# yilunliao/vit-search

Hardware: AMD Instinct MI355X
Metric: images/sec/node ViT-ResNAS-Tiny supernet train, bs128/GPU, 1/2/4/8 MI355X (higher is better)
Workload: dtype bf16

## Files before the change

vit-search_amd/csrc/attn_mfma.hip:

```cpp
#include <cstdlib>

#include "common.h"
#include "../../include/vitres_hip.h"

namespace vr_attn_mfma {

typedef __bf16 bfv8 __attribute__((ext_vector_type(8)));

template <int D> struct AC {
    static constexpr int NCH = D / 8;
    static constexpr int DK = (D + 31) / 32;
    static constexpr int DT = D / 16;
    static constexpr bool SWZ = (D != 48);
};

template <typename TI = bf16_t> __device__ __forceinline__ f32x4 mfma16(bfv8 a, bfv8 b, f32x4 c) { return Half16<TI>::mfma16(a, b, c); }

template <int D, int MAXNP, int NTHR>
__device__ __forceinline__ void stage_chunked(char* dst, const bf16_t* __restrict__ src, int rs, int N, int Np, int tid) {
    const int NpS = Np + 8;
    constexpr int NCH = AC<D>::NCH, HP = NCH / 2;
    constexpr int IT = (MAXNP * NCH + NTHR - 1) / NTHR;
    const int total = Np * NCH;
    uint4 v[IT];
// ... 71 lines not shown
    __device__ static __forceinline__ int tbase(int lane) {
        const int g = lane >> 4, i = lane & 15;
        return ((((i & 3) >> 1)) * (NP + 8) + 4 * g + (i >> 2)) * 16 + (i & 1) * 8;
    }
    __device__ static __forceinline__ const char* opaque(const char* p) {
        typedef __attribute__((address_space(3))) const char lds_char;
        unsigned a = (unsigned)(unsigned long long)(lds_char*)p;
        asm volatile("" : "+v"(a));
        return (const char*)(lds_char*)(unsigned long long)a;
    }
    __device__ static __forceinline__ bfv8 cread(const char* lane_base, int row0) {
        return *reinterpret_cast<const bfv8*>(lane_base + row0 * 16);
    }
    __device__ static __forceinline__ bfv8 tread(const char* lane_base, int kp, int dt) {
        typedef __attribute__((address_space(3))) s4v lds_s4v;
        const char* p = lane_base + (2 * dt * (NP + 8) + 32 * kp) * 16;
        const s4v lo = __builtin_amdgcn_ds_read_tr16_b64_v4i16((lds_s4v*)(p));
        const s4v hi = __builtin_amdgcn_ds_read_tr16_b64_v4i16((lds_s4v*)(p + 16 * 16));
        const s8v v = {lo[0], lo[1], lo[2], lo[3], hi[0], hi[1], hi[2], hi[3]};
        return __builtin_bit_cast(bfv8, v);
    }
};

template <int D, int NKP, int NW, int PB, int OCC, bool FULL, typename TI = bf16_t>
__global__ __launch_bounds__(NW * 64, OCC) void fwd_kernel(const bf16_t* __restrict__ qkv, bf16_t* __restrict__ o,
                                                           float* __restrict__ lse, const int* __restrict__ keep_hd, int B,
                                                           int N, int H, float scale, int ATTN_XCD) {
    static_assert(NKP % PB == 0, "key-tile pairs must split into whole blocks");
    constexpr int NP = 32 * NKP;
    typedef Img<D, NP> I;
    extern __shared__ __attribute__((aligned(16))) char sm[];
    const int bidx = xcd_block((int)blockIdx.x, (int)gridDim.x, ATTN_XCD);
    const int b = bidx / H, h = bidx % H;
    const int tid = threadIdx.x, lane = tid & 63, wave = tid >> 6, g = lane >> 4, c = lane & 15;
    const int HD = H * D, RS = 3 * HD;
    const bf16_t* base = qkv + (long long)b * N * RS + h * D;
    bf16_t* ob = o + (long long)b * N * HD + h * D;
    float* lb = lse + ((long long)b * H + h) * N;
    if (keep_hd && h * D >= keep_hd[b]) {
        for (int i = tid; i < N * (D / 8); i += NW * 64) {
            const int n = i / (D / 8), ch = i % (D / 8);
            *reinterpret_cast<uint4*>(ob + (long long)n * HD + ch * 8) = make_uint4(0, 0, 0, 0);
        }
        for (int n = tid; n < N; n += NW * 64) lb[n] = 0.f;
        return;
    }
    char* Kc = sm;
    char* Vc = sm + I::BYTES;
    int q0 = wave * 16;
    bfv8 qf[AC<D>::DK];
#pragma unroll
    for (int dk = 0; dk < AC<D>::DK; ++dk) qf[dk] = gfrag<D>(base, RS, q0, N, dk, lane);
    stage_chunked<D, NP, NW * 64>(Kc, base + HD, RS, N, NP, tid);
    stage_chunked<D, NP, NW * 64>(Vc, base + 2 * HD, RS, N, NP, tid);
    __syncthreads();
    const char* kb[AC<D>::DK];
#pragma unroll
    for (int dk = 0; dk < AC<D>::DK; ++dk) kb[dk] = I::opaque(Kc + I::cbase(dk, lane));
    const char* vb = I::opaque(Vc + I::tbase(lane));
    const float cs = scale * LOG2E;
    while (q0 < N) {
        float m = -INFINITY, sum = 0.f;
        f32x4 oacc[AC<D>::DT];
#pragma unroll
        for (int dt = 0; dt < AC<D>::DT; ++dt) oacc[dt] = f32x4{0.f, 0.f, 0.f, 0.f};
#pragma unroll
        for (int b0 = 0; b0 < NKP; b0 += PB) {
            if (FULL || b0 * 32 < N) {
                f32x4 st[2 * PB];
                float bm = -INFINITY;
#pragma unroll
                for (int j = 0; j < 2 * PB; ++j) {
                    const int k0 = (2 * b0 + j) * 16;
                    f32x4 acc = {0.f, 0.f, 0.f, 0.f};
                    if (FULL || k0 < N) {
#pragma unroll
                        for (int dk = 0; dk < AC<D>::DK; ++dk) acc = mfma16<TI>(I::cread(kb[dk], k0), qf[dk], acc);
                        if (FULL ? (2 * b0 + j >= 2 * NKP - 2) : (k0 + 16 > N)) {
#pragma unroll
                            for (int r = 0; r < 4; ++r) acc[r] = (k0 + 4 * g + r) < N ? acc[r] : -INFINITY;
                        }
                    } else {
                        acc = f32x4{-INFINITY, -INFINITY, -INFINITY, -INFINITY};
                    }
                    st[j] = acc;
                    bm = fmaxf(fmaxf(bm, fmaxf(acc[0], acc[1])), fmaxf(acc[2], acc[3]));
                }
                bm = gmax(bm);
                const float mn = fmaxf(m, bm);
                const float alpha = ex2((m - mn) * cs);
                const float mc = mn * cs;
                float ps = 0.f;
#pragma unroll
                for (int j = 0; j < 2 * PB; ++j)
#pragma unroll
                    for (int r = 0; r < 4; ++r) {
                        const float pv = ex2(fmaf(st[j][r], cs, -mc));
                        st[j][r] = pv;
                        ps += pv;
                    }
                sum = sum * alpha + ps;
                m = mn;
                if (b0 > 0) {
#pragma unroll
                    for (int dt = 0; dt < AC<D>::DT; ++dt)
#pragma unroll
                        for (int r = 0; r < 4; ++r) oacc[dt][r] *= alpha;
                }
#pragma unroll
                for (int jp = 0; jp < PB; ++jp) {
                    if (FULL || (b0 + jp) * 32 < N) {
                        const bfv8 pf = pack8<TI>(st[2 * jp], st[2 * jp + 1]);
#pragma unroll
                        for (int dt = 0; dt < AC<D>::DT; ++dt) oacc[dt] = mfma16<TI>(I::tread(vb, b0 + jp, dt), pf, oacc[dt]);
                    }
                }
                __builtin_amdgcn_sched_barrier(0);
            }
        }
        sum = gsum(sum);
        const float inv = 1.0f / sum;
        const int qs = q0;
        q0 += NW * 16;
        bfv8 qn[AC<D>::DK];
        if (q0 < N) {
#pragma unroll
            for (int dk = 0; dk < AC<D>::DK; ++dk) qn[dk] = gfrag<D>(base, RS, q0, N, dk, lane);
        }
        if (qs + c < N) {
#pragma unroll
            for (int dt = 0; dt < AC<D>::DT; ++dt)
                *reinterpret_cast<uint2*>(ob + (long long)(qs + c) * HD + dt * 16 + 4 * g) =
                    make_uint2(Half16<TI>::pk(oacc[dt][0] * inv, oacc[dt][1] * inv), Half16<TI>::pk(oacc[dt][2] * inv, oacc[dt][3] * inv));
            if (g == 0) lb[qs + c] = m * scale + __logf(sum);
        }
        if (q0 < N) {
#pragma unroll
            for (int dk = 0; dk < AC<D>::DK; ++dk) qf[dk] = qn[dk];
        }
    }
}

template <int D, int NKP, int NW, int OCC, bool FULL>
__global__ __launch_bounds__(NW * 64, OCC) void bwd_dq_kernel(const bf16_t* __restrict__ qkv, const bf16_t* __restrict__ o,
                                                              const bf16_t* __restrict__ d_o, const float* __restrict__ lse,
                                                              float* __restrict__ delta, bf16_t* __restrict__ dqkv,
                                                              const int* __restrict__ keep_hd, int B, int N, int H,
                                                              float scale, int ATTN_XCD) {
    constexpr int NP = 32 * NKP;
    typedef Img<D, NP> I;
    extern __shared__ __attribute__((aligned(16))) char sm[];
    const int bidx = xcd_block((int)blockIdx.x, (int)gridDim.x, ATTN_XCD);
    const int b = bidx / H, h = bidx % H;
    const int tid = threadIdx.x, lane = tid & 63, wave = tid >> 6, g = lane >> 4, c = lane & 15;
    const int HD = H * D, RS = 3 * HD;
    const bf16_t* base = qkv + (long long)b * N * RS + h * D;
    bf16_t* dbase = dqkv + (long long)b * N * RS + h * D;
    if (keep_hd && h * D >= keep_hd[b]) {
        for (int i = tid; i < N * (D / 8); i += NW * 64) {
            const int n = i / (D / 8), ch = i % (D / 8);
            *reinterpret_cast<uint4*>(dbase + (long long)n * RS + ch * 8) = make_uint4(0, 0, 0, 0);
        }
        return;
    }
    const bf16_t* ob = o + (long long)b * N * HD + h * D;
    const bf16_t* gb = d_o + (long long)b * N * HD + h * D;
    const float* lb = lse + ((long long)b * H + h) * N;
    float* db = delta + ((long long)b * H + h) * N;
    char* Kc = sm;
    char* Vc = Kc + I::BYTES;
    int q0 = wave * 16;
    bfv8 qf[AC<D>::DK], gf[AC<D>::DK], of[AC<D>::DK];
    float lq = 0.f;
#pragma unroll
    for (int dk = 0; dk < AC<D>::DK; ++dk) {
        qf[dk] = gfrag<D>(base, RS, q0, N, dk, lane);
        gf[dk] = gfrag<D>(gb, HD, q0, N, dk, lane);
        of[dk] = gfrag<D>(ob, HD, q0, N, dk, lane);
    }
    if (q0 + c < N) lq = lb[q0 + c];
    stage_chunked<D, NP, NW * 64>(Kc, base + HD, RS, N, NP, tid);
    stage_chunked<D, NP, NW * 64>(Vc, base + 2 * HD, RS, N, NP, tid);
    __syncthreads();
    const char *kb[AC<D>::DK], *vb[AC<D>::DK];
#pragma unroll
    for (int dk = 0; dk < AC<D>::DK; ++dk) {
        kb[dk] = I::opaque(Kc + I::cbase(dk, lane));
        vb[dk] = I::opaque(Vc + I::cbase(dk, lane));
    }
    const char* kt_b = I::opaque(Kc + I::tbase(lane));
    const float cs = scale * LOG2E;
    while (q0 < N) {
        float d = 0.f;
#pragma unroll
        for (int dk = 0; dk < AC<D>::DK; ++dk)
#pragma unroll
            for (int e = 0; e < 8; ++e) d += (float)gf[dk][e] * (float)of[dk][e];
        const float dl = gsum(d);
        const float l2 = lq * LOG2E;
        if (g == 0 && q0 + c < N) db[q0 + c] = dl;
        f32x4 dq[AC<D>::DT];
#pragma unroll
        for (int dt = 0; dt < AC<D>::DT; ++dt) dq[dt] = f32x4{0.f, 0.f, 0.f, 0.f};
#pragma unroll
        for (int kp = 0; kp < NKP; ++kp) {
            if (FULL || kp * 32 < N) {
                f32x4 ds[2];
#pragma unroll
                for (int tt = 0; tt < 2; ++tt) {
                    const int k0 = (2 * kp + tt) * 16;
                    f32x4 sc = {0.f, 0.f, 0.f, 0.f}, dp = {0.f, 0.f, 0.f, 0.f};
                    if (FULL || k0 < N) {
#pragma unroll
                        for (int dk = 0; dk < AC<D>::DK; ++dk) {
                            sc = mfma16(I::cread(kb[dk], k0), qf[dk], sc);
                            dp = mfma16(I::cread(vb[dk], k0), gf[dk], dp);
                        }
#pragma unroll
                        for (int r = 0; r < 4; ++r) sc[r] = ex2(fmaf(sc[r], cs, -l2)) * ((dp[r] - dl) * scale);
                    }
                    ds[tt] = sc;
                }
                const bfv8 sf = pack8(ds[0], ds[1]);
#pragma unroll
                for (int dt = 0; dt < AC<D>::DT; ++dt) dq[dt] = mfma16(I::tread(kt_b, kp, dt), sf, dq[dt]);
                if (kp % 3 == 2) __builtin_amdgcn_sched_barrier(0);
            }
        }
        const int qs = q0;
        q0 += NW * 16;
        if (q0 < N) {
#pragma unroll
            for (int dk = 0; dk < AC<D>::DK; ++dk) {
                qf[dk] = gfrag<D>(base, RS, q0, N, dk, lane);
                gf[dk] = gfrag<D>(gb, HD, q0, N, dk, lane);
                of[dk] = gfrag<D>(ob, HD, q0, N, dk, lane);
            }
            lq = q0 + c < N ? lb[q0 + c] : 0.f;
        }
        if (qs + c < N) {
#pragma unroll
            for (int dt = 0; dt < AC<D>::DT; ++dt)
                *reinterpret_cast<uint2*>(dbase + (long long)(qs + c) * RS + dt * 16 + 4 * g) =
                    make_uint2(pack_bf2(dq[dt][0], dq[dt][1]), pack_bf2(dq[dt][2], dq[dt][3]));
        }
    }
}

template <int D, int NKP, int NW, int OCC, bool FULL>
__global__ __launch_bounds__(NW * 64, OCC) void bwd_dkv_kernel(const bf16_t* __restrict__ qkv, const bf16_t* __restrict__ d_o,
                                                               const float* __restrict__ lse, const float* __restrict__ delta,
                                                               bf16_t* __restrict__ dqkv, const int* __restrict__ keep_hd,
                                                               int B, int N, int H, float scale, int ATTN_XCD) {
    constexpr int NP = 32 * NKP;
    typedef Img<D, NP> I;
    extern __shared__ __attribute__((aligned(16))) char sm[];
    const int bidx = xcd_block((int)blockIdx.x, (int)gridDim.x, ATTN_XCD);
    const int b = bidx / H, h = bidx % H;
    const int tid = threadIdx.x, lane = tid & 63, wave = tid >> 6, g = lane >> 4, c = lane & 15;
    const int HD = H * D, RS = 3 * HD;
    const bf16_t* base = qkv + (long long)b * N * RS + h * D;
    bf16_t* dbase = dqkv + (long long)b * N * RS + h * D;
    if (keep_hd && h * D >= keep_hd[b]) {
        for (int i = tid; i < N * (D / 8); i += NW * 64) {
            const int n = i / (D / 8), ch = i % (D / 8);
            *reinterpret_cast<uint4*>(dbase + (long long)n * RS + HD + ch * 8) = make_uint4(0, 0, 0, 0);
            *reinterpret_cast<uint4*>(dbase + (long long)n * RS + 2 * HD + ch * 8) = make_uint4(0, 0, 0, 0);
        }
        return;
    }
    const bf16_t* gb = d_o + (long long)b * N * HD + h * D;
    const int nqp = FULL ? NKP : (N + 31) / 32;
    char* Qc = sm;
    char* Gc = Qc + I::BYTES;
    float* Ls = reinterpret_cast<float*>(Gc + I::BYTES);
    float* Ds = Ls + NP;
    int u0 = wave * 16;
    bfv8 kf[AC<D>::DK], vf[AC<D>::DK];
#pragma unroll
    for (int dk = 0; dk < AC<D>::DK; ++dk) {
        kf[dk] = gfrag<D>(base + HD, RS, u0, N, dk, lane);
        vf[dk] = gfrag<D>(base + 2 * HD, RS, u0, N, dk, lane);
    }
    for (int n = tid; n < NP; n += NW * 64) {
        Ls[n] = n < N ? lse[((long long)b * H + h) * N + n] * LOG2E : 0.f;
        Ds[n] = n < N ? delta[((long long)b * H + h) * N + n] : 0.f;
    }
    stage_chunked<D, NP, NW * 64>(Qc, base, RS, N, NP, tid);
    stage_chunked<D, NP, NW * 64>(Gc, gb, HD, N, NP, tid);
    __syncthreads();
    const char *qb[AC<D>::DK], *gcb[AC<D>::DK];
#pragma unroll
    for (int dk = 0; dk < AC<D>::DK; ++dk) {
        qb[dk] = I::opaque(Qc + I::cbase(dk, lane));
        gcb[dk] = I::opaque(Gc + I::cbase(dk, lane));
    }
    const char* qt_b = I::opaque(Qc + I::tbase(lane));
    const char* gt_b = I::opaque(Gc + I::tbase(lane));
    const float* lsg = Ls + 4 * g;
    const float* dsg = Ds + 4 * g;
    const float cs = scale * LOG2E;
    while (u0 < N) {
        f32x4 dka[AC<D>::DT], dva[AC<D>::DT];
#pragma unroll
        for (int dt = 0; dt < AC<D>::DT; ++dt) {
            dka[dt] = f32x4{0.f, 0.f, 0.f, 0.f};
            dva[dt] = f32x4{0.f, 0.f, 0.f, 0.f};
        }
#pragma unroll(NKP <= 3 ? NKP : 1)
        for (int qp = 0; qp < nqp; ++qp) {
            f32x4 p[2], ds[2];
#pragma unroll
            for (int tt = 0; tt < 2; ++tt) {
                const int q0 = qp * 32 + tt * 16;
                const float4 l4 = *reinterpret_cast<const float4*>(lsg + q0);
                const float4 d4 = *reinterpret_cast<const float4*>(dsg + q0);
                const float lr[4] = {l4.x, l4.y, l4.z, l4.w}, dr[4] = {d4.x, d4.y, d4.z, d4.w};
                f32x4 sc = {0.f, 0.f, 0.f, 0.f}, dp = {0.f, 0.f, 0.f, 0.f};
#pragma unroll
                for (int dk = 0; dk < AC<D>::DK; ++dk) {
                    sc = mfma16(I::cread(qb[dk], q0), kf[dk], sc);
                    dp = mfma16(I::cread(gcb[dk], q0), vf[dk], dp);
                }
#pragma unroll
                for (int r = 0; r < 4; ++r) {
                    const float pv = ex2(fmaf(sc[r], cs, -lr[r]));
                    p[tt][r] = pv;
                    ds[tt][r] = pv * ((dp[r] - dr[r]) * scale);
                }
            }
            const bfv8 pf = pack8(p[0], p[1]), sf = pack8(ds[0], ds[1]);
#pragma unroll
            for (int dt = 0; dt < AC<D>::DT; ++dt) {
                dva[dt] = mfma16(I::tread(gt_b, qp, dt), pf, dva[dt]);
                dka[dt] = mfma16(I::tread(qt_b, qp, dt), sf, dka[dt]);
            }
            __builtin_amdgcn_sched_barrier(0);
        }
        const int k = u0 + c;
        u0 += NW * 16;
        if (u0 < N) {
#pragma unroll
            for (int dk = 0; dk < AC<D>::DK; ++dk) {
                kf[dk] = gfrag<D>(base + HD, RS, u0, N, dk, lane);
                vf[dk] = gfrag<D>(base + 2 * HD, RS, u0, N, dk, lane);
            }
        }
        if (k < N) {
#pragma unroll
            for (int dt = 0; dt < AC<D>::DT; ++dt) {
                bf16_t* dst = dbase + (long long)k * RS + dt * 16 + 4 * g;
                *reinterpret_cast<uint2*>(dst + HD) =
                    make_uint2(pack_bf2(dka[dt][0], dka[dt][1]), pack_bf2(dka[dt][2], dka[dt][3]));
                *reinterpret_cast<uint2*>(dst + 2 * HD) =
                    make_uint2(pack_bf2(dva[dt][0], dva[dt][1]), pack_bf2(dva[dt][2], dva[dt][3]));
            }
        }
    }
}

template <int D, int MAXNP, int NTHR>
__device__ __forceinline__ void stage_load(uint4 (&v)[(MAXNP * AC<D>::NCH + NTHR - 1) / NTHR], const bf16_t* __restrict__ src, int rs,
                                           int N, int Np, int tid) {
    constexpr int NCH = AC<D>::NCH, HP = NCH / 2;
    constexpr int IT = (MAXNP * NCH + NTHR - 1) / NTHR;
    const int total = Np * NCH;
#pragma unroll
    for (int it = 0; it < IT; ++it) {
        const int idx = tid + it * NTHR;
        const int q = idx >> 3, l8 = idx & 7;
        const int rb = q / HP, cp = q - rb * HP;
        const int n = 4 * rb + (l8 >> 1), ch = 2 * cp + (l8 & 1);
        const bool ok = n < N && idx < total;
        v[it] = *reinterpret_cast<const uint4*>(src + (long long)(ok ? n : 0) * rs + (ok ? ch : 0) * 8);
        if (!ok) v[it] = make_uint4(0, 0, 0, 0);
    }
}
template <int D, int MAXNP, int NTHR>
__device__ __forceinline__ void stage_store(char* dst, const uint4 (&v)[(MAXNP * AC<D>::NCH + NTHR - 1) / NTHR], int Np, int tid) {
    const int NpS = Np + 8;
    constexpr int NCH = AC<D>::NCH, HP = NCH / 2;
    constexpr int IT = (MAXNP * NCH + NTHR - 1) / NTHR;
    const int total = Np * NCH;
#pragma unroll
    for (int it = 0; it < IT; ++it) {
        const int idx = tid + it * NTHR;
        const int q = idx >> 3, l8 = idx & 7;
        const int rb = q / HP, cp = q - rb * HP;
        const int n = 4 * rb + (l8 >> 1), ch = 2 * cp + (l8 & 1);
        if (idx < total) *reinterpret_cast<uint4*>(dst + ((size_t)ch * NpS + n) * 16) = v[it];
    }
}

template <int D, int NKP, int NW, int OCC, bool FULL>
__global__ __launch_bounds__(NW * 64, OCC) void bwd_short_kernel(const bf16_t* __restrict__ qkv, const bf16_t* __restrict__ o,
                                                                 const bf16_t* __restrict__ d_o, const float* __restrict__ lse,
                                                                 float* __restrict__ delta, bf16_t* __restrict__ dqkv,
                                                                 const int* __restrict__ keep_hd, int B, int N, int H,
                                                                 float scale, int ATTN_XCD) {
    constexpr int NP = 32 * NKP, NT = NW * 64;
    constexpr int IT = (NP * AC<D>::NCH + NT - 1) / NT;
    typedef Img<D, NP> I;
    extern __shared__ __attribute__((aligned(16))) char sm[];
    const int bidx = xcd_block((int)blockIdx.x, (int)gridDim.x, ATTN_XCD);
    const int b = bidx / H, h = bidx % H;
    const int tid = threadIdx.x, lane = tid & 63, wave = tid >> 6, g = lane >> 4, c = lane & 15;
    const int HD = H * D, RS = 3 * HD;
    const bf16_t* base = qkv + (long long)b * N * RS + h * D;
    bf16_t* dbase = dqkv + (long long)b * N * RS + h * D;
    if (keep_hd && h * D >= keep_hd[b]) {
        for (int i = tid; i < N * (D / 8); i += NT) {
            const int n = i / (D / 8), ch = i % (D / 8);
            bf16_t* dst = dbase + (long long)n * RS + ch * 8;
            *reinterpret_cast<uint4*>(dst) = make_uint4(0, 0, 0, 0);
            *reinterpret_cast<uint4*>(dst + HD) = make_uint4(0, 0, 0, 0);
            *reinterpret_cast<uint4*>(dst + 2 * HD) = make_uint4(0, 0, 0, 0);
        }
        return;
    }
    const bf16_t* ob = o + (long long)b * N * HD + h * D;
    const bf16_t* gb = d_o + (long long)b * N * HD + h * D;
    const float* lb = lse + ((long long)b * H + h) * N;
// ... 24 lines not shown
        stage_store<D, NP, NT>(Gc, vg, NP, tid);
    }
    __syncthreads();
    const char *qb[AC<D>::DK], *kb[AC<D>::DK], *vb[AC<D>::DK], *gcb[AC<D>::DK];
#pragma unroll
    for (int dk = 0; dk < AC<D>::DK; ++dk) {
        qb[dk] = I::opaque(Qc + I::cbase(dk, lane));
        kb[dk] = I::opaque(Kc + I::cbase(dk, lane));
        vb[dk] = I::opaque(Vc + I::cbase(dk, lane));
        gcb[dk] = I::opaque(Gc + I::cbase(dk, lane));
    }
    const char* kt_b = I::opaque(Kc + I::tbase(lane));
    const char* qt_b = I::opaque(Qc + I::tbase(lane));
    const char* gt_b = I::opaque(Gc + I::tbase(lane));
    const float cs = scale * LOG2E;
    auto zfrag = [&](const char* lane_base, int row0, int dk) -> bfv8 {
        bfv8 v = I::cread(lane_base, row0);
        if constexpr (AC<D>::NCH % 4 != 0) {
            if (dk * 4 + (lane >> 4) >= AC<D>::NCH) v = __builtin_bit_cast(bfv8, make_uint4(0, 0, 0, 0));
        }
        return v;
    };

    while (q0 < N) {
        bfv8 qf[AC<D>::DK], gf[AC<D>::DK];
#pragma unroll
        for (int dk = 0; dk < AC<D>::DK; ++dk) {
            qf[dk] = zfrag(qb[dk], q0, dk);
            gf[dk] = zfrag(gcb[dk], q0, dk);
        }
        float d = 0.f;
#pragma unroll
        for (int dk = 0; dk < AC<D>::DK; ++dk)
#pragma unroll
            for (int e = 0; e < 8; ++e) d += (float)gf[dk][e] * (float)of[dk][e];
        const float dl = gsum(d);
        const float l2 = Ls[q0 + c];
        if (g == 0 && q0 + c < N) {
            db[q0 + c] = dl;
            Ds[q0 + c] = dl;
        }
        f32x4 dq[AC<D>::DT];
#pragma unroll
        for (int dt = 0; dt < AC<D>::DT; ++dt) dq[dt] = f32x4{0.f, 0.f, 0.f, 0.f};
#pragma unroll
        for (int kp = 0; kp < NKP; ++kp) {
            if (FULL || kp * 32 < N) {
                f32x4 ds[2];
#pragma unroll
                for (int tt = 0; tt < 2; ++tt) {
                    const int k0 = (2 * kp + tt) * 16;
                    f32x4 sc = {0.f, 0.f, 0.f, 0.f}, dp = {0.f, 0.f, 0.f, 0.f};
                    if (FULL || k0 < N) {
#pragma unroll
                        for (int dk = 0; dk < AC<D>::DK; ++dk) {
                            sc = mfma16(I::cread(kb[dk], k0), qf[dk], sc);
                            dp = mfma16(I::cread(vb[dk], k0), gf[dk], dp);
                        }
#pragma unroll
                        for (int r = 0; r < 4; ++r) sc[r] = ex2(fmaf(sc[r], cs, -l2)) * ((dp[r] - dl) * scale);
                    }
                    ds[tt] = sc;
                }
                const bfv8 sf = pack8(ds[0], ds[1]);
#pragma unroll
                for (int dt = 0; dt < AC<D>::DT; ++dt) dq[dt] = mfma16(I::tread(kt_b, kp, dt), sf, dq[dt]);
                __builtin_amdgcn_sched_barrier(0);
            }
        }
        const int qs = q0;
        q0 += NW * 16;
        if (q0 < N) {
#pragma unroll
            for (int dk = 0; dk < AC<D>::DK; ++dk) of[dk] = gfrag<D>(ob, HD, q0, N, dk, lane);
        }
        if (qs + c < N) {
#pragma unroll
            for (int dt = 0; dt < AC<D>::DT; ++dt)
                *reinterpret_cast<uint2*>(dbase + (long long)(qs + c) * RS + dt * 16 + 4 * g) =
                    make_uint2(pack_bf2(dq[dt][0], dq[dt][1]), pack_bf2(dq[dt][2], dq[dt][3]));
        }
    }
    __syncthreads();

    const int nqp = FULL ? NKP : (N + 31) / 32;
    const float* lsg = Ls + 4 * g;
    const float* dsg = Ds + 4 * g;
    for (int u0 = wave * 16; u0 < N; u0 += NW * 16) {
        bfv8 kf[AC<D>::DK], vf[AC<D>::DK];
#pragma unroll
        for (int dk = 0; dk < AC<D>::DK; ++dk) {
            kf[dk] = zfrag(kb[dk], u0, dk);
            vf[dk] = zfrag(vb[dk], u0, dk);
        }
        f32x4 dka[AC<D>::DT], dva[AC<D>::DT];
#pragma unroll
        for (int dt = 0; dt < AC<D>::DT; ++dt) {
            dka[dt] = f32x4{0.f, 0.f, 0.f, 0.f};
            dva[dt] = f32x4{0.f, 0.f, 0.f, 0.f};
        }
#pragma unroll
        for (int qp = 0; qp < NKP; ++qp) {
            if (qp < nqp) {
                f32x4 p[2], ds[2];
#pragma unroll
                for (int tt = 0; tt < 2; ++tt) {
                    const int qq = qp * 32 + tt * 16;
                    const float4 l4 = *reinterpret_cast<const float4*>(lsg + qq);
                    const float4 d4 = *reinterpret_cast<const float4*>(dsg + qq);
                    const float lr[4] = {l4.x, l4.y, l4.z, l4.w}, dr[4] = {d4.x, d4.y, d4.z, d4.w};
                    f32x4 sc = {0.f, 0.f, 0.f, 0.f}, dp = {0.f, 0.f, 0.f, 0.f};
#pragma unroll
                    for (int dk = 0; dk < AC<D>::DK; ++dk) {
                        sc = mfma16(I::cread(qb[dk], qq), kf[dk], sc);
                        dp = mfma16(I::cread(gcb[dk], qq), vf[dk], dp);
                    }
#pragma unroll
                    for (int r = 0; r < 4; ++r) {
                        const float pv = ex2(fmaf(sc[r], cs, -lr[r]));
                        p[tt][r] = pv;
                        ds[tt][r] = pv * ((dp[r] - dr[r]) * scale);
                    }
                }
                const bfv8 pf = pack8(p[0], p[1]), sf = pack8(ds[0], ds[1]);
#pragma unroll
                for (int dt = 0; dt < AC<D>::DT; ++dt) {
                    dva[dt] = mfma16(I::tread(gt_b, qp, dt), pf, dva[dt]);
                    dka[dt] = mfma16(I::tread(qt_b, qp, dt), sf, dka[dt]);
                }
                __builtin_amdgcn_sched_barrier(0);
            }
        }
        const int k = u0 + c;
        if (k < N) {
#pragma unroll
            for (int dt = 0; dt < AC<D>::DT; ++dt) {
                bf16_t* dst = dbase + (long long)k * RS + dt * 16 + 4 * g;
                *reinterpret_cast<uint2*>(dst + HD) =
                    make_uint2(pack_bf2(dka[dt][0], dka[dt][1]), pack_bf2(dka[dt][2], dka[dt][3]));
                *reinterpret_cast<uint2*>(dst + 2 * HD) =
                    make_uint2(pack_bf2(dva[dt][0], dva[dt][1]), pack_bf2(dva[dt][2], dva[dt][3]));
            }
        }
    }
}

constexpr int LKB = 256, LQB = 128, LNW = 8;

template <int D, typename TI = bf16_t>
__global__ __launch_bounds__(LNW * 64) void fwd_long_kernel(const bf16_t* __restrict__ qkv, bf16_t* __restrict__ o,
                                                            float* __restrict__ lse, const int* __restrict__ keep_hd, int B,
                                                            int N, int H, float scale) {
    extern __shared__ __attribute__((aligned(16))) char sm[];
    const int nqb = (N + LQB - 1) / LQB;
    const int qb = blockIdx.x % nqb, bh = blockIdx.x / nqb, b = bh / H, h = bh % H;
    const int tid = threadIdx.x, lane = tid & 63, wave = tid >> 6, g = lane >> 4, c = lane & 15;
    const int HD = H * D, RS = 3 * HD;
    const bf16_t* base = qkv + (long long)b * N * RS + h * D;
    bf16_t* ob = o + (long long)b * N * HD + h * D;
    float* lb = lse + ((long long)b * H + h) * N;
    const int q0 = qb * LQB + wave * 16;
    if (keep_hd && h * D >= keep_hd[b]) {
        for (int i = tid; i < LQB * (D / 8); i += LNW * 64) {
            const int n = qb * LQB + i / (D / 8), ch = i % (D / 8);
            if (n < N) *reinterpret_cast<uint4*>(ob + (long long)n * HD + ch * 8) = make_uint4(0, 0, 0, 0);
        }
// ... 249 lines not shown
            *reinterpret_cast<uint2*>(dst + 2 * HD) = make_uint2(pack_bf2(dva[dt][0], dva[dt][1]), pack_bf2(dva[dt][2], dva[dt][3]));
        }
    }
}

template <typename K> static int set_lds(K kernel, size_t bytes) {
    static size_t granted = 0;
    if (bytes > 64 * 1024 && bytes > granted) {
        hipError_t e = hipFuncSetAttribute(reinterpret_cast<const void*>(kernel), hipFuncAttributeMaxDynamicSharedMemorySize,
                                           (int)bytes);
        if (e != hipSuccess) return (int)e;
        granted = bytes;
    }
    return 0;
}

template <int NKP> struct Plan {
    static constexpr int NW = NKP >= 9 ? 8 : 4;
    static constexpr int OCC = 4;
    static constexpr int PB = NKP >= 9 ? 3 : NKP;
};

static constexpr int attn_xcd() { return 1; }
template <int D, int NKP, typename TI = bf16_t>
static int launch_fwd(const bf16_t* qkv, bf16_t* o, float* lse, const int* keep, int B, int N, int H, float scale,
                      hipStream_t st) {
    constexpr int NW = Plan<NKP>::NW, OCC = Plan<NKP>::OCC, PB = Plan<NKP>::PB;
    const size_t lds = (size_t)2 * Img<D, 32 * NKP>::BYTES;
    if (N > 32 * (NKP - 1)) {
        int rc = set_lds(fwd_kernel<D, NKP, NW, PB, OCC, true, TI>, lds);
        if (rc) return rc;
        hipLaunchKernelGGL((fwd_kernel<D, NKP, NW, PB, OCC, true, TI>), dim3(B * H), dim3(NW * 64), lds, st, qkv, o, lse, keep, B, N, H,
                           scale, attn_xcd());
    } else {
        int rc = set_lds(fwd_kernel<D, NKP, NW, PB, OCC, false, TI>, lds);
        if (rc) return rc;
        hipLaunchKernelGGL((fwd_kernel<D, NKP, NW, PB, OCC, false, TI>), dim3(B * H), dim3(NW * 64), lds, st, qkv, o, lse, keep, B, N, H,
                           scale, attn_xcd());
    }
    return 0;
}
template <int D, int NKP>
static int launch_bwd(const bf16_t* qkv, const bf16_t* o, const bf16_t* d_o, const float* lse, float* delta, bf16_t* dqkv,
                      const int* keep, int B, int N, int H, float scale, hipStream_t st) {
    constexpr int NW = Plan<NKP>::NW, OCC = Plan<NKP>::OCC;
    const size_t l1 = (size_t)2 * Img<D, 32 * NKP>::BYTES, l2 = l1 + 2 * 32 * NKP * sizeof(float);
    {
        constexpr size_t L3 = (size_t)4 * Img<D, 32 * NKP>::BYTES + 2 * 32 * NKP * sizeof(float);
        constexpr int SOCC = NKP <= 3 ? 3 : (L3 <= 80 * 1024 ? 2 : 1);
        const bool merged = SOCC >= 2;
        if (merged) {
            const size_t l3 = (size_t)4 * Img<D, 32 * NKP>::BYTES + 2 * 32 * NKP * sizeof(float);
            if (N > 32 * (NKP - 1)) {
                int rc = set_lds(bwd_short_kernel<D, NKP, NW, SOCC, true>, l3);
                if (rc) return rc;
                hipLaunchKernelGGL((bwd_short_kernel<D, NKP, NW, SOCC, true>), dim3(B * H), dim3(NW * 64), l3, st, qkv, o, d_o, lse, delta,
                                   dqkv, keep, B, N, H, scale, attn_xcd());
            } else {
                int rc = set_lds(bwd_short_kernel<D, NKP, NW, SOCC, false>, l3);
                if (rc) return rc;
                hipLaunchKernelGGL((bwd_short_kernel<D, NKP, NW, SOCC, false>), dim3(B * H), dim3(NW * 64), l3, st, qkv, o, d_o, lse, delta,
                                   dqkv, keep, B, N, H, scale, attn_xcd());
            }
            return 0;
        }
    }
    if (N > 32 * (NKP - 1)) {
        int rc = set_lds(bwd_dq_kernel<D, NKP, NW, OCC, true>, l1);
        if (rc) return rc;
        rc = set_lds(bwd_dkv_kernel<D, NKP, NW, OCC, true>, l2);
        if (rc) return rc;
        hipLaunchKernelGGL((bwd_dq_kernel<D, NKP, NW, OCC, true>), dim3(B * H), dim3(NW * 64), l1, st, qkv, o, d_o, lse, delta, dqkv,
                           keep, B, N, H, scale, attn_xcd());
        hipLaunchKernelGGL((bwd_dkv_kernel<D, NKP, NW, OCC, true>), dim3(B * H), dim3(NW * 64), l2, st, qkv, d_o, lse, delta, dqkv,
                           keep, B, N, H, scale, attn_xcd());
    } else {
        int rc = set_lds(bwd_dq_kernel<D, NKP, NW, OCC, false>, l1);
        if (rc) return rc;
        rc = set_lds(bwd_dkv_kernel<D, NKP, NW, OCC, false>, l2);
        if (rc) return rc;
        hipLaunchKernelGGL((bwd_dq_kernel<D, NKP, NW, OCC, false>), dim3(B * H), dim3(NW * 64), l1, st, qkv, o, d_o, lse, delta, dqkv,
                           keep, B, N, H, scale, attn_xcd());
        hipLaunchKernelGGL((bwd_dkv_kernel<D, NKP, NW, OCC, false>), dim3(B * H), dim3(NW * 64), l2, st, qkv, d_o, lse, delta, dqkv,
                           keep, B, N, H, scale, attn_xcd());
    }
    return 0;
}

template <int D, typename TI = bf16_t>
static int launch_fwd_long(const bf16_t* qkv, bf16_t* o, float* lse, const int* keep, int B, int N, int H, float scale,
                           hipStream_t st) {
    const size_t lds = (size_t)2 * D * (LKB + 8) * 2;
    int rc = set_lds(fwd_long_kernel<D, TI>, lds);
    if (rc) return rc;
    hipLaunchKernelGGL((fwd_long_kernel<D, TI>), dim3(B * H * ((N + LQB - 1) / LQB)), dim3(LNW * 64), lds, st, qkv, o, lse, keep, B, N, H,
                       scale);
    return 0;
}
template <int D>
static int launch_bwd_long(const bf16_t* qkv, const bf16_t* o, const bf16_t* d_o, const float* lse, float* delta, bf16_t* dqkv,
                           const int* keep, int B, int N, int H, float scale, hipStream_t st) {
    const size_t l1 = (size_t)2 * D * (LKB + 8) * 2, l2 = l1 + 2 * LKB * sizeof(float);
    int rc = set_lds(bwd_dq_long_kernel<D>, l1);
    if (rc) return rc;
    rc = set_lds(bwd_dkv_long_kernel<D>, l2);
    if (rc) return rc;
    const unsigned grid = (unsigned)(B * H * ((N + LQB - 1) / LQB));
    hipLaunchKernelGGL((bwd_dq_long_kernel<D>), dim3(grid), dim3(LNW * 64), l1, st, qkv, o, d_o, lse, delta, dqkv, keep, B, N, H, scale);
// ... 62 lines not shown
```

Baseline: 18660.

## Specialize attention kernels for partial last key tile and single-row tail

Adds MODE template specializations for the attention forward and backward kernels based on how many rows fall in the last 32-wide tile. When that tile holds at most 16 rows, the upper 16-row half is skipped entirely. When only one row is left (e.g. a CLS token making N = 32k+1), that row is handled by a dedicated tail path split across waves and reduced through LDS, so the main loop stops at a 16-aligned boundary. This removes wasted MFMA and exp work on padded tiles, at the cost of extra syncthreads, LDS reductions and more template instances.

New measurement: 18640. No clear change (-0.1%).

```diff
diff --git a/vit-search_amd/csrc/attn_mfma.hip b/vit-search_amd/csrc/attn_mfma.hip
--- a/vit-search_amd/csrc/attn_mfma.hip
+++ b/vit-search_amd/csrc/attn_mfma.hip
@@ -1,4 +1,5 @@
 #include <cstdlib>
+#include <type_traits>
 
 #include "common.h"
 #include "../../include/vitres_hip.h"
@@ -117,11 +118,102 @@
     }
 };
 
-template <int D, int NKP, int NW, int PB, int OCC, bool FULL, typename TI = bf16_t>
+template <int MODE> struct Mode {
+    static constexpr bool FULL = MODE >= 1, HALF = MODE >= 2, TAIL = MODE == 3;
+};
+template <int D, int NROW>
+__device__ __forceinline__ void tail_put(float* P, int wave, int slot, const f32x4 (&acc)[AC<D>::DT], int g, int c) {
+    if (c == 0) {
+#pragma unroll
+        for (int dt = 0; dt < AC<D>::DT; ++dt)
+            *reinterpret_cast<float4*>(P + (wave * NROW + slot) * D + dt * 16 + 4 * g) = make_float4(acc[dt][0], acc[dt][1], acc[dt][2], acc[dt][3]);
+    }
+}
+template <int D, int NROW, int NW>
+__device__ __forceinline__ void tail_sum_store(const float* P, bf16_t* dst, int sst, int tid) {
+    if (tid < NROW * D / 2) {
+        const int slot = tid / (D / 2), d = 2 * (tid % (D / 2));
+        float a0 = 0.f, a1 = 0.f;
+#pragma unroll
+        for (int w = 0; w < NW; ++w) {
+            const float2 v = *reinterpret_cast<const float2*>(P + (w * NROW + slot) * D + d);
+            a0 += v.x;
+            a1 += v.y;
+        }
+        *reinterpret_cast<uint32_t*>(dst + slot * sst + d) = pack_bf2(a0, a1);
+    }
+}
+template <int D, int NKP, int NW, typename I>
+__device__ __forceinline__ void tail_dq(f32x4 (&dq)[AC<D>::DT], const bfv8 (&qf)[AC<D>::DK], const bfv8 (&gf)[AC<D>::DK], float l2, float dl,
+                                        const char* const (&kb)[AC<D>::DK], const char* const (&vb)[AC<D>::DK], const char* kt_b,
+                                        float cs, float scale, int wave) {
+    for (int kp = wave; kp < NKP; kp += NW) {
+        f32x4 ds[2];
+#pragma unroll
+        for (int tt = 0; tt < 2; ++tt) {
+            f32x4 sc = {0.f, 0.f, 0.f, 0.f}, dp = {0.f, 0.f, 0.f, 0.f};
+            if (tt == 0 || kp != NKP - 1) {
+                const int k0 = (2 * kp + tt) * 16;
+#pragma unroll
+                for (int dk = 0; dk < AC<D>::DK; ++dk) {
+                    sc = mfma16(I::cread(kb[dk], k0), qf[dk], sc);
+                    dp = mfma16(I::cread(vb[dk], k0), gf[dk], dp);
+                }
+#pragma unroll
+                for (int r = 0; r < 4; ++r) sc[r] = ex2(fmaf(sc[r], cs, -l2)) * ((dp[r] - dl) * scale);
+            }
+            ds[tt] = sc;
+        }
+        const bfv8 sf = pack8(ds[0], ds[1]);
+#pragma unroll
+        for (int dt = 0; dt < AC<D>::DT; ++dt) dq[dt] = mfma16(I::tread(kt_b, kp, dt), sf, dq[dt]);
+    }
+}
+template <int D, int NKP, int NW, typename I>
+__device__ __forceinline__ void tail_dkv(f32x4 (&dka)[AC<D>::DT], f32x4 (&dva)[AC<D>::DT], const bfv8 (&kf)[AC<D>::DK],
+                                         const bfv8 (&vf)[AC<D>::DK], const char* const (&qb)[AC<D>::DK],
+                                         const char* const (&gcb)[AC<D>::DK], const char* qt_b, const char* gt_b, const float* lsg,
+                                         const float* dsg, float cs, float scale, int wave) {
+    for (int qp = wave; qp < NKP; qp += NW) {
+        f32x4 p[2], ds[2];
+#pragma unroll
+        for (int tt = 0; tt < 2; ++tt) {
+            p[tt] = f32x4{0.f, 0.f, 0.f, 0.f};
+            ds[tt] = f32x4{0.f, 0.f, 0.f, 0.f};
+            if (tt == 0 || qp != NKP - 1) {
+                const int q0 = qp * 32 + tt * 16;
+                const float4 l4 = *reinterpret_cast<const float4*>(lsg + q0);
+                const float4 d4 = *reinterpret_cast<const float4*>(dsg + q0);
+                const float lr[4] = {l4.x, l4.y, l4.z, l4.w}, dr[4] = {d4.x, d4.y, d4.z, d4.w};
+                f32x4 sc = {0.f, 0.f, 0.f, 0.f}, dp = {0.f, 0.f, 0.f, 0.f};
+#pragma unroll
+                for (int dk = 0; dk < AC<D>::DK; ++dk) {
+                    sc = mfma16(I::cread(qb[dk], q0), kf[dk], sc);
+                    dp = mfma16(I::cread(gcb[dk], q0), vf[dk], dp);
+                }
+#pragma unroll
+                for (int r = 0; r < 4; ++r) {
+                    const float pv = ex2(fmaf(sc[r], cs, -lr[r]));
+                    p[tt][r] = pv;
+                    ds[tt][r] = pv * ((dp[r] - dr[r]) * scale);
+                }
+            }
+        }
+        const bfv8 pf = pack8(p[0], p[1]), sf = pack8(ds[0], ds[1]);
+#pragma unroll
+        for (int dt = 0; dt < AC<D>::DT; ++dt) {
+            dva[dt] = mfma16(I::tread(gt_b, qp, dt), pf, dva[dt]);
+            dka[dt] = mfma16(I::tread(qt_b, qp, dt), sf, dka[dt]);
+        }
+    }
+}
+
+template <int D, int NKP, int NW, int PB, int OCC, int MODE, typename TI = bf16_t>
 __global__ __launch_bounds__(NW * 64, OCC) void fwd_kernel(const bf16_t* __restrict__ qkv, bf16_t* __restrict__ o,
                                                            float* __restrict__ lse, const int* __restrict__ keep_hd, int B,
                                                            int N, int H, float scale, int ATTN_XCD) {
     static_assert(NKP % PB == 0, "key-tile pairs must split into whole blocks");
+    constexpr bool FULL = Mode<MODE>::FULL, HALF = Mode<MODE>::HALF, TAIL = Mode<MODE>::TAIL;
     constexpr int NP = 32 * NKP;
     typedef Img<D, NP> I;
     extern __shared__ __attribute__((aligned(16))) char sm[];
@@ -154,7 +246,8 @@
     for (int dk = 0; dk < AC<D>::DK; ++dk) kb[dk] = I::opaque(Kc + I::cbase(dk, lane));
     const char* vb = I::opaque(Vc + I::tbase(lane));
     const float cs = scale * LOG2E;
-    while (q0 < N) {
+    const int NE = TAIL ? N - 1 : N;
+    while (q0 < NE) {
         float m = -INFINITY, sum = 0.f;
         f32x4 oacc[AC<D>::DT];
 #pragma unroll
@@ -168,10 +261,14 @@
                 for (int j = 0; j < 2 * PB; ++j) {
                     const int k0 = (2 * b0 + j) * 16;
                     f32x4 acc = {0.f, 0.f, 0.f, 0.f};
+                    if (HALF && 2 * b0 + j == 2 * NKP - 1) {
+                        st[j] = acc;
+                        continue;
+                    }
                     if (FULL || k0 < N) {
 #pragma unroll
                         for (int dk = 0; dk < AC<D>::DK; ++dk) acc = mfma16<TI>(I::cread(kb[dk], k0), qf[dk], acc);
-                        if (FULL ? (2 * b0 + j >= 2 * NKP - 2) : (k0 + 16 > N)) {
+                        if (HALF ? (2 * b0 + j == 2 * NKP - 2) : FULL ? (2 * b0 + j >= 2 * NKP - 2) : (k0 + 16 > N)) {
 #pragma unroll
                             for (int r = 0; r < 4; ++r) acc[r] = (k0 + 4 * g + r) < N ? acc[r] : -INFINITY;
                         }
@@ -187,13 +284,15 @@
                 const float mc = mn * cs;
                 float ps = 0.f;
 #pragma unroll
-                for (int j = 0; j < 2 * PB; ++j)
+                for (int j = 0; j < 2 * PB; ++j) {
+                    if (HALF && 2 * b0 + j == 2 * NKP - 1) continue;
 #pragma unroll
                     for (int r = 0; r < 4; ++r) {
                         const float pv = ex2(fmaf(st[j][r], cs, -mc));
                         st[j][r] = pv;
                         ps += pv;
                     }
+                }
                 sum = sum * alpha + ps;
                 m = mn;
                 if (b0 > 0) {
@@ -218,7 +317,7 @@
         const int qs = q0;
         q0 += NW * 16;
         bfv8 qn[AC<D>::DK];
-        if (q0 < N) {
+        if (q0 < NE) {
 #pragma unroll
             for (int dk = 0; dk < AC<D>::DK; ++dk) qn[dk] = gfrag<D>(base, RS, q0, N, dk, lane);
         }
@@ -229,19 +328,96 @@
                     make_uint2(Half16<TI>::pk(oacc[dt][0] * inv, oacc[dt][1] * inv), Half16<TI>::pk(oacc[dt][2] * inv, oacc[dt][3] * inv));
             if (g == 0) lb[qs + c] = m * scale + __logf(sum);
         }
-        if (q0 < N) {
+        if (q0 < NE) {
 #pragma unroll
             for (int dk = 0; dk < AC<D>::DK; ++dk) qf[dk] = qn[dk];
         }
     }
-}
-
-template <int D, int NKP, int NW, int OCC, bool FULL>
+    if constexpr (TAIL) {
+#pragma unroll
+        for (int dk = 0; dk < AC<D>::DK; ++dk) qf[dk] = gfrag<D>(base, RS, N - 1, N, dk, lane);
+        float m = -INFINITY, sum = 0.f;
+        f32x4 oacc[AC<D>::DT];
+#pragma unroll
+        for (int dt = 0; dt < AC<D>::DT; ++dt) oacc[dt] = f32x4{0.f, 0.f, 0.f, 0.f};
+        for (int kp = wave; kp < NKP; kp += NW) {
+            f32x4 s0 = {0.f, 0.f, 0.f, 0.f}, s1 = {0.f, 0.f, 0.f, 0.f};
+            const bool last = kp == NKP - 1;
+#pragma unroll
+            for (int dk = 0; dk < AC<D>::DK; ++dk) s0 = mfma16<TI>(I::cread(kb[dk], 32 * kp), qf[dk], s0);
+            float bm;
+            if (last) {
+#pragma unroll
+                for (int r = 0; r < 4; ++r) s0[r] = (32 * kp + 4 * g + r) < N ? s0[r] : -INFINITY;
+                bm = fmaxf(fmaxf(s0[0], s0[1]), fmaxf(s0[2], s0[3]));
+            } else {
+#pragma unroll
+                for (int dk = 0; dk < AC<D>::DK; ++dk) s1 = mfma16<TI>(I::cread(kb[dk], 32 * kp + 16), qf[dk], s1);
+                bm = fmaxf(fmaxf(fmaxf(s0[0], s0[1]), fmaxf(s0[2], s0[3])), fmaxf(fmaxf(s1[0], s1[1]), fmaxf(s1[2], s1[3])));
+            }
+            bm = gmax(bm);
+            const float mn = fmaxf(m, bm);
+            const float alpha = ex2((m - mn) * cs);
+            const float mc = mn * cs;
+            float ps = 0.f;
+#pragma unroll
+            for (int r = 0; r < 4; ++r) {
+                s0[r] = ex2(fmaf(s0[r], cs, -mc));
+                ps += s0[r];
+            }
+            if (!last) {
+#pragma unroll
+                for (int r = 0; r < 4; ++r) {
+                    s1[r] = ex2(fmaf(s1[r], cs, -mc));
+                    ps += s1[r];
+                }
+            }
+            sum = sum * alpha + ps;
+            m = mn;
+#pragma unroll
+            for (int dt = 0; dt < AC<D>::DT; ++dt)
+#pragma unroll
+                for (int r = 0; r < 4; ++r) oacc[dt][r] *= alpha;
+            const bfv8 pf = pack8<TI>(s0, s1);
+#pragma unroll
+            for (int dt = 0; dt < AC<D>::DT; ++dt) oacc[dt] = mfma16<TI>(I::tread(vb, kp, dt), pf, oacc[dt]);
+        }
+        sum = gsum(sum);
+        float* P = reinterpret_cast<float*>(sm);
+        __syncthreads();
+        tail_put<D, 1>(P, wave, 0, oacc, g, c);
+        if (lane == 0) {
+            P[NW * D + wave] = m;
+            P[NW * D + NW + wave] = sum;
+        }
+        __syncthreads();
+        if (tid < D / 2) {
+            float mx = P[NW * D];
+#pragma unroll
+            for (int w = 1; w < NW; ++w) mx = fmaxf(mx, P[NW * D + w]);
+            float tot = 0.f, a0 = 0.f, a1 = 0.f;
+#pragma unroll
+            for (int w = 0; w < NW; ++w) {
+                const float a = ex2((P[NW * D + w] - mx) * cs);
+                const float2 v = *reinterpret_cast<const float2*>(P + w * D + 2 * tid);
+                tot += a * P[NW * D + NW + w];
+                a0 += a * v.x;
+                a1 += a * v.y;
+            }
+            const float inv = 1.0f / tot;
+            *reinterpret_cast<uint32_t*>(ob + (long long)(N - 1) * HD + 2 * tid) = Half16<TI>::pk(a0 * inv, a1 * inv);
+            if (tid == 0) lb[N - 1] = mx * scale + __logf(tot);
+        }
+    }
+}
+
+template <int D, int NKP, int NW, int OCC, int MODE>
 __global__ __launch_bounds__(NW * 64, OCC) void bwd_dq_kernel(const bf16_t* __restrict__ qkv, const bf16_t* __restrict__ o,
                                                               const bf16_t* __restrict__ d_o, const float* __restrict__ lse,
                                                               float* __restrict__ delta, bf16_t* __restrict__ dqkv,
                                                               const int* __restrict__ keep_hd, int B, int N, int H,
                                                               float scale, int ATTN_XCD) {
+    constexpr bool FULL = Mode<MODE>::FULL, HALF = Mode<MODE>::HALF, TAIL = Mode<MODE>::TAIL;
     constexpr int NP = 32 * NKP;
     typedef Img<D, NP> I;
     extern __shared__ __attribute__((aligned(16))) char sm[];
@@ -285,7 +461,8 @@
     }
     const char* kt_b = I::opaque(Kc + I::tbase(lane));
     const float cs = scale * LOG2E;
-    while (q0 < N) {
+    const int NE = TAIL ? N - 1 : N;
+    while (q0 < NE) {
         float d = 0.f;
 #pragma unroll
         for (int dk = 0; dk < AC<D>::DK; ++dk)
@@ -305,7 +482,7 @@
                 for (int tt = 0; tt < 2; ++tt) {
                     const int k0 = (2 * kp + tt) * 16;
                     f32x4 sc = {0.f, 0.f, 0.f, 0.f}, dp = {0.f, 0.f, 0.f, 0.f};
-                    if (FULL || k0 < N) {
+                    if ((FULL || k0 < N) && !(HALF && 2 * kp + tt == 2 * NKP - 1)) {
 #pragma unroll
                         for (int dk = 0; dk < AC<D>::DK; ++dk) {
                             sc = mfma16(I::cread(kb[dk], k0), qf[dk], sc);
@@ -324,7 +501,7 @@
         }
         const int qs = q0;
         q0 += NW * 16;
-        if (q0 < N) {
+        if (q0 < NE) {
 #pragma unroll
             for (int dk = 0; dk < AC<D>::DK; ++dk) {
                 qf[dk] = gfrag<D>(base, RS, q0, N, dk, lane);
@@ -340,13 +517,39 @@
                     make_uint2(pack_bf2(dq[dt][0], dq[dt][1]), pack_bf2(dq[dt][2], dq[dt][3]));
         }
     }
-}
-
-template <int D, int NKP, int NW, int OCC, bool FULL>
+    if constexpr (TAIL) {
+#pragma unroll
+        for (int dk = 0; dk < AC<D>::DK; ++dk) {
+            qf[dk] = gfrag<D>(base, RS, N - 1, N, dk, lane);
+            gf[dk] = gfrag<D>(gb, HD, N - 1, N, dk, lane);
+            of[dk] = gfrag<D>(ob, HD, N - 1, N, dk, lane);
+        }
+        lq = c == 0 ? lb[N - 1] : 0.f;
+        float d = 0.f;
+#pragma unroll
+        for (int dk = 0; dk < AC<D>::DK; ++dk)
+#pragma unroll
+            for (int e = 0; e < 8; ++e) d += (float)gf[dk][e] * (float)of[dk][e];
+        const float dl = gsum(d);
+        if (wave == 0 && lane == 0) db[N - 1] = dl;
+        f32x4 dq[AC<D>::DT];
+#pragma unroll
+        for (int dt = 0; dt < AC<D>::DT; ++dt) dq[dt] = f32x4{0.f, 0.f, 0.f, 0.f};
+        tail_dq<D, NKP, NW, I>(dq, qf, gf, lq * LOG2E, dl, kb, vb, kt_b, cs, scale, wave);
+        float* P = reinterpret_cast<float*>(sm);
+        __syncthreads();
+        tail_put<D, 1>(P, wave, 0, dq, g, c);
+        __syncthreads();
+        tail_sum_store<D, 1, NW>(P, dbase + (long long)(N - 1) * RS, 0, tid);
+    }
+}
+
+template <int D, int NKP, int NW, int OCC, int MODE>
 __global__ __launch_bounds__(NW * 64, OCC) void bwd_dkv_kernel(const bf16_t* __restrict__ qkv, const bf16_t* __restrict__ d_o,
                                                                const float* __restrict__ lse, const float* __restrict__ delta,
                                                                bf16_t* __restrict__ dqkv, const int* __restrict__ keep_hd,
                                                                int B, int N, int H, float scale, int ATTN_XCD) {
+    constexpr bool FULL = Mode<MODE>::FULL, HALF = Mode<MODE>::HALF, TAIL = Mode<MODE>::TAIL;
     constexpr int NP = 32 * NKP;
     typedef Img<D, NP> I;
     extern __shared__ __attribute__((aligned(16))) char sm[];
@@ -365,7 +568,7 @@
         return;
     }
     const bf16_t* gb = d_o + (long long)b * N * HD + h * D;
-    const int nqp = FULL ? NKP : (N + 31) / 32;
+    const int nqp = HALF ? NKP - 1 : FULL ? NKP : (N + 31) / 32;
     char* Qc = sm;
     char* Gc = Qc + I::BYTES;
     float* Ls = reinterpret_cast<float*>(Gc + I::BYTES);
@@ -395,18 +598,23 @@
     const float* lsg = Ls + 4 * g;
     const float* dsg = Ds + 4 * g;
     const float cs = scale * LOG2E;
-    while (u0 < N) {
+    const int NE = TAIL ? N - 1 : N;
+    while (u0 < NE) {
         f32x4 dka[AC<D>::DT], dva[AC<D>::DT];
 #pragma unroll
         for (int dt = 0; dt < AC<D>::DT; ++dt) {
             dka[dt] = f32x4{0.f, 0.f, 0.f, 0.f};
             dva[dt] = f32x4{0.f, 0.f, 0.f, 0.f};
         }
-#pragma unroll(NKP <= 3 ? NKP : 1)
-        for (int qp = 0; qp < nqp; ++qp) {
+        auto pair = [&](int qp, auto half) {
             f32x4 p[2], ds[2];
 #pragma unroll
             for (int tt = 0; tt < 2; ++tt) {
+                if (decltype(half)::value && tt == 1) {
+                    p[tt] = f32x4{0.f, 0.f, 0.f, 0.f};
+                    ds[tt] = f32x4{0.f, 0.f, 0.f, 0.f};
+                    continue;
+                }
                 const int q0 = qp * 32 + tt * 16;
                 const float4 l4 = *reinterpret_cast<const float4*>(lsg + q0);
                 const float4 d4 = *reinterpret_cast<const float4*>(dsg + q0);
@@ -431,10 +639,13 @@
                 dka[dt] = mfma16(I::tread(qt_b, qp, dt), sf, dka[dt]);
             }
             __builtin_amdgcn_sched_barrier(0);
-        }
+        };
+#pragma unroll(NKP <= 3 ? NKP : 1)
+        for (int qp = 0; qp < nqp; ++qp) pair(qp, std::false_type{});
+        if constexpr (HALF) pair(NKP - 1, std::true_type{});
         const int k = u0 + c;
         u0 += NW * 16;
-        if (u0 < N) {
+        if (u0 < NE) {
 #pragma unroll
             for (int dk = 0; dk < AC<D>::DK; ++dk) {
                 kf[dk] = gfrag<D>(base + HD, RS, u0, N, dk, lane);
@@ -451,6 +662,26 @@
                     make_uint2(pack_bf2(dva[dt][0], dva[dt][1]), pack_bf2(dva[dt][2], dva[dt][3]));
             }
         }
+    }
+    if constexpr (TAIL) {
+#pragma unroll
+        for (int dk = 0; dk < AC<D>::DK; ++dk) {
+            kf[dk] = gfrag<D>(base + HD, RS, N - 1, N, dk, lane);
+            vf[dk] = gfrag<D>(base + 2 * HD, RS, N - 1, N, dk, lane);
+        }
+        f32x4 dka[AC<D>::DT], dva[AC<D>::DT];
+#pragma unroll
+        for (int dt = 0; dt < AC<D>::DT; ++dt) {
+            dka[dt] = f32x4{0.f, 0.f, 0.f, 0.f};
+            dva[dt] = f32x4{0.f, 0.f, 0.f, 0.f};
+        }
+        tail_dkv<D, NKP, NW, I>(dka, dva, kf, vf, qb, gcb, qt_b, gt_b, lsg, dsg, cs, scale, wave);
+        float* P = reinterpret_cast<float*>(sm);
+        __syncthreads();
+        tail_put<D, 2>(P, wave, 0, dka, g, c);
+        tail_put<D, 2>(P, wave, 1, dva, g, c);
+        __syncthreads();
+        tail_sum_store<D, 2, NW>(P, dbase + (long long)(N - 1) * RS + HD, HD, tid);
     }
 }
 
@@ -487,12 +718,13 @@
     }
 }
 
-template <int D, int NKP, int NW, int OCC, bool FULL>
+template <int D, int NKP, int NW, int OCC, int MODE>
 __global__ __launch_bounds__(NW * 64, OCC) void bwd_short_kernel(const bf16_t* __restrict__ qkv, const bf16_t* __restrict__ o,
                                                                  const bf16_t* __restrict__ d_o, const float* __restrict__ lse,
                                                                  float* __restrict__ delta, bf16_t* __restrict__ dqkv,
                                                                  const int* __restrict__ keep_hd, int B, int N, int H,
                                                                  float scale, int ATTN_XCD) {
+    constexpr bool FULL = Mode<MODE>::FULL, HALF = Mode<MODE>::HALF, TAIL = Mode<MODE>::TAIL;
     constexpr int NP = 32 * NKP, NT = NW * 64;
     constexpr int IT = (NP * AC<D>::NCH + NT - 1) / NT;
     typedef Img<D, NP> I;
@@ -563,7 +795,8 @@
         return v;
     };
 
-    while (q0 < N) {
+    const int NE = TAIL ? N - 1 : N;
+    while (q0 < NE) {
         bfv8 qf[AC<D>::DK], gf[AC<D>::DK];
 #pragma unroll
         for (int dk = 0; dk < AC<D>::DK; ++dk) {
@@ -592,7 +825,7 @@
                 for (int tt = 0; tt < 2; ++tt) {
                     const int k0 = (2 * kp + tt) * 16;
                     f32x4 sc = {0.f, 0.f, 0.f, 0.f}, dp = {0.f, 0.f, 0.f, 0.f};
-                    if (FULL || k0 < N) {
+                    if ((FULL || k0 < N) && !(HALF && 2 * kp + tt == 2 * NKP - 1)) {
 #pragma unroll
                         for (int dk = 0; dk < AC<D>::DK; ++dk) {
                             sc = mfma16(I::cread(kb[dk], k0), qf[dk], sc);
@@ -611,7 +844,7 @@
         }
         const int qs = q0;
         q0 += NW * 16;
-        if (q0 < N) {
+        if (q0 < NE) {
 #pragma unroll
             for (int dk = 0; dk < AC<D>::DK; ++dk) of[dk] = gfrag<D>(ob, HD, q0, N, dk, lane);
         }
@@ -622,12 +855,35 @@
                     make_uint2(pack_bf2(dq[dt][0], dq[dt][1]), pack_bf2(dq[dt][2], dq[dt][3]));
         }
     }
+    f32x4 tq[AC<D>::DT], tk[AC<D>::DT], tv[AC<D>::DT];
+    if constexpr (TAIL) {
+        bfv8 qf[AC<D>::DK], gf[AC<D>::DK];
+#pragma unroll
+        for (int dk = 0; dk < AC<D>::DK; ++dk) {
+            of[dk] = gfrag<D>(ob, HD, N - 1, N, dk, lane);
+            qf[dk] = zfrag(qb[dk], N - 1, dk);
+            gf[dk] = zfrag(gcb[dk], N - 1, dk);
+        }
+        float d = 0.f;
+#pragma unroll
+        for (int dk = 0; dk < AC<D>::DK; ++dk)
+#pragma unroll
+            for (int e = 0; e < 8; ++e) d += (float)gf[dk][e] * (float)of[dk][e];
+        const float dl = gsum(d);
+        if (wave == 0 && lane == 0) {
+            db[N - 1] = dl;
+            Ds[N - 1] = dl;
+        }
+#pragma unroll
+        for (int dt = 0; dt < AC<D>::DT; ++dt) tq[dt] = f32x4{0.f, 0.f, 0.f, 0.f};
+        tail_dq<D, NKP, NW, I>(tq, qf, gf, Ls[N - 1 + c], dl, kb, vb, kt_b, cs, scale, wave);
+    }
     __syncthreads();
 
     const int nqp = FULL ? NKP : (N + 31) / 32;
     const float* lsg = Ls + 4 * g;
     const float* dsg = Ds + 4 * g;
-    for (int u0 = wave * 16; u0 < N; u0 += NW * 16) {
+    for (int u0 = wave * 16; u0 < NE; u0 += NW * 16) {
         bfv8 kf[AC<D>::DK], vf[AC<D>::DK];
 #pragma unroll
         for (int dk = 0; dk < AC<D>::DK; ++dk) {
@@ -646,6 +902,11 @@
                 f32x4 p[2], ds[2];
 #pragma unroll
                 for (int tt = 0; tt < 2; ++tt) {
+                    if (HALF && qp == NKP - 1 && tt == 1) {
+                        p[tt] = f32x4{0.f, 0.f, 0.f, 0.f};
+                        ds[tt] = f32x4{0.f, 0.f, 0.f, 0.f};
+                        continue;
+                    }
                     const int qq = qp * 32 + tt * 16;
                     const float4 l4 = *reinterpret_cast<const float4*>(lsg + qq);
                     const float4 d4 = *reinterpret_cast<const float4*>(dsg + qq);
@@ -683,6 +944,27 @@
                     make_uint2(pack_bf2(dva[dt][0], dva[dt][1]), pack_bf2(dva[dt][2], dva[dt][3]));
             }
         }
+    }
+    if constexpr (TAIL) {
+        bfv8 kf[AC<D>::DK], vf[AC<D>::DK];
+#pragma unroll
+        for (int dk = 0; dk < AC<D>::DK; ++dk) {
+            kf[dk] = zfrag(kb[dk], N - 1, dk);
+            vf[dk] = zfrag(vb[dk], N - 1, dk);
+        }
+#pragma unroll
+        for (int dt = 0; dt < AC<D>::DT; ++dt) {
+            tk[dt] = f32x4{0.f, 0.f, 0.f, 0.f};
+            tv[dt] = f32x4{0.f, 0.f, 0.f, 0.f};
+        }
+        tail_dkv<D, NKP, NW, I>(tk, tv, kf, vf, qb, gcb, qt_b, gt_b, lsg, dsg, cs, scale, wave);
+        float* P = reinterpret_cast<float*>(sm);
+        __syncthreads();
+        tail_put<D, 3>(P, wave, 0, tq, g, c);
+        tail_put<D, 3>(P, wave, 1, tk, g, c);
+        tail_put<D, 3>(P, wave, 2, tv, g, c);
+        __syncthreads();
+        tail_sum_store<D, 3, NW>(P, dbase + (long long)(N - 1) * RS, HD, tid);
     }
 }
 
@@ -978,22 +1260,28 @@
 };
 
 static constexpr int attn_xcd() { return 1; }
+static int attn_mode(int N, int NKP) {
+    const int r = N - 32 * (NKP - 1);
+    return r <= 0 ? 0 : r > 16 ? 1 : (r == 1 && NKP > 1) ? 3 : 2;
+}
+#define VR_ATTN_MODE(N, NKP, M, ...)                                        \
+    switch (attn_mode(N, NKP)) {                                            \
+        case 0: { constexpr int M = 0; __VA_ARGS__ } break;                 \
+        case 1: { constexpr int M = 1; __VA_ARGS__ } break;                 \
+        case 2: { constexpr int M = 2; __VA_ARGS__ } break;                 \
+        default: { constexpr int M = (NKP > 1 ? 3 : 2); __VA_ARGS__ } break; \
+    }
 template <int D, int NKP, typename TI = bf16_t>
 static int launch_fwd(const bf16_t* qkv, bf16_t* o, float* lse, const int* keep, int B, int N, int H, float scale,
                       hipStream_t st) {
     constexpr int NW = Plan<NKP>::NW, OCC = Plan<NKP>::OCC, PB = Plan<NKP>::PB;
     const size_t lds = (size_t)2 * Img<D, 32 * NKP>::BYTES;
-    if (N > 32 * (NKP - 1)) {
-        int rc = set_lds(fwd_kernel<D, NKP, NW, PB, OCC, true, TI>, lds);
+    VR_ATTN_MODE(N, NKP, M, {
+        int rc = set_lds(fwd_kernel<D, NKP, NW, PB, OCC, M, TI>, lds);
         if (rc) return rc;
-        hipLaunchKernelGGL((fwd_kernel<D, NKP, NW, PB, OCC, true, TI>), dim3(B * H), dim3(NW * 64), lds, st, qkv, o, lse, keep, B, N, H,
+        hipLaunchKernelGGL((fwd_kernel<D, NKP, NW, PB, OCC, M, TI>), dim3(B * H), dim3(NW * 64), lds, st, qkv, o, lse, keep, B, N, H,
                            scale, attn_xcd());
-    } else {
-        int rc = set_lds(fwd_kernel<D, NKP, NW, PB, OCC, false, TI>, lds);
-        if (rc) return rc;
-        hipLaunchKernelGGL((fwd_kernel<D, NKP, NW, PB, OCC, false, TI>), dim3(B * H), dim3(NW * 64), lds, st, qkv, o, lse, keep, B, N, H,
-                           scale, attn_xcd());
-    }
+    })
     return 0;
 }
 template <int D, int NKP>
@@ -1007,39 +1295,25 @@
         const bool merged = SOCC >= 2;
         if (merged) {
             const size_t l3 = (size_t)4 * Img<D, 32 * NKP>::BYTES + 2 * 32 * NKP * sizeof(float);
-            if (N > 32 * (NKP - 1)) {
-                int rc = set_lds(bwd_short_kernel<D, NKP, NW, SOCC, true>, l3);
+            VR_ATTN_MODE(N, NKP, M, {
+                int rc = set_lds(bwd_short_kernel<D, NKP, NW, SOCC, M>, l3);
                 if (rc) return rc;
-                hipLaunchKernelGGL((bwd_short_kernel<D, NKP, NW, SOCC, true>), dim3(B * H), dim3(NW * 64), l3, st, qkv, o, d_o, lse, delta,
+                hipLaunchKernelGGL((bwd_short_kernel<D, NKP, NW, SOCC, M>), dim3(B * H), dim3(NW * 64), l3, st, qkv, o, d_o, lse, delta,
                                    dqkv, keep, B, N, H, scale, attn_xcd());
-            } else {
-                int rc = set_lds(bwd_short_kernel<D, NKP, NW, SOCC, false>, l3);
-                if (rc) return rc;
-                hipLaunchKernelGGL((bwd_short_kernel<D, NKP, NW, SOCC, false>), dim3(B * H), dim3(NW * 64), l3, st, qkv, o, d_o, lse, delta,
-                                   dqkv, keep, B, N, H, scale, attn_xcd());
-            }
+            })
             return 0;
         }
     }
-    if (N > 32 * (NKP - 1)) {
-        int rc = set_lds(bwd_dq_kernel<D, NKP, NW, OCC, true>, l1);
+    VR_ATTN_MODE(N, NKP, M, {
+        int rc = set_lds(bwd_dq_kernel<D, NKP, NW, OCC, M>, l1);
         if (rc) return rc;
-        rc = set_lds(bwd_dkv_kernel<D, NKP, NW, OCC, true>, l2);
+        rc = set_lds(bwd_dkv_kernel<D, NKP, NW, OCC, M>, l2);
         if (rc) return rc;
-        hipLaunchKernelGGL((bwd_dq_kernel<D, NKP, NW, OCC, true>), dim3(B * H), dim3(NW * 64), l1, st, qkv, o, d_o, lse, delta, dqkv,
+        hipLaunchKernelGGL((bwd_dq_kernel<D, NKP, NW, OCC, M>), dim3(B * H), dim3(NW * 64), l1, st, qkv, o, d_o, lse, delta, dqkv,
                            keep, B, N, H, scale, attn_xcd());
-        hipLaunchKernelGGL((bwd_dkv_kernel<D, NKP, NW, OCC, true>), dim3(B * H), dim3(NW * 64), l2, st, qkv, d_o, lse, delta, dqkv,
+        hipLaunchKernelGGL((bwd_dkv_kernel<D, NKP, NW, OCC, M>), dim3(B * H), dim3(NW * 64), l2, st, qkv, d_o, lse, delta, dqkv,
                            keep, B, N, H, scale, attn_xcd());
-    } else {
-        int rc = set_lds(bwd_dq_kernel<D, NKP, NW, OCC, false>, l1);
-        if (rc) return rc;
-        rc = set_lds(bwd_dkv_kernel<D, NKP, NW, OCC, false>, l2);
-        if (rc) return rc;
-        hipLaunchKernelGGL((bwd_dq_kernel<D, NKP, NW, OCC, false>), dim3(B * H), dim3(NW * 64), l1, st, qkv, o, d_o, lse, delta, dqkv,
-                           keep, B, N, H, scale, attn_xcd());
-        hipLaunchKernelGGL((bwd_dkv_kernel<D, NKP, NW, OCC, false>), dim3(B * H), dim3(NW * 64), l2, st, qkv, d_o, lse, delta, dqkv,
-                           keep, B, N, H, scale, attn_xcd());
-    }
+    })
     return 0;
 }
 
```
